# tjsdn3065/Practice_path_planning_for_formula_student_driverless

Hardware: AMD Instinct MI355X
Metric: PGD outer-iters/sec (N=2000 samples, closed, competition_map1, 1024 alpha-seeds/GPU, min-curv) (higher is better)
Workload: dtype f64; 1 GPU; C2: competition_map1 closed, N=2000, B=1024 alpha-seeds per GPU, min-curvature, 14 outer iterations, default cfg::Config; N=2000, batch_per_gpu=1024, global_batch=1024, parallelism=dp1: one GPU, no collective

## Files before the change

### practice_path_planning_for_formula_student_driverless_amd/csrc/rl_optimize_body.inc

```
    constexpr int NW = T / 64;
    constexpr bool WARM = WarmStart<T, MT>::value;
    __shared__ Smem<K, T, WARM> sm;
#ifdef RL_STAMPS
    unsigned long long st_acc[16] = {};
    unsigned long long st_last = __builtin_amdgcn_s_memtime();
#endif

    const int tid = threadIdx.x, lane = tid & 63, wid = tid >> 6;
    const int N = p.N;
    const int base = tid * K;
    const int Ta = (N + K - 1) / K;
    const bool active = tid < Ta;
    const int cnt = RAGGED ? min(K, max(0, N - base)) : (tid < Ta ? K : 0);
    const int cntL = N - (Ta - 1) * K;
    const int wid_u = __builtin_amdgcn_readfirstlane(wid);
    const bool part_wave = RAGGED && (cntL != K) && (((Ta - 1) >> 6) == wid_u);
    const bool tail_wave = wid_u >= ((Ta - 1) >> 6);
    constexpr bool OPEN_FAST = !CLOSED && !RAGGED && K >= 4;
    const bool edge_wave = OPEN_FAST && (wid_u == 0 || wid_u == ((Ta - 1) >> 6));
    const bool fl = tid == 0, ll = tid == Ta - 1;
    const rl_cfg& C = p.cfg[p.ncfg == 1 ? 0 : b];
    const uint64_t seed = p.seeds ? p.seeds[b] : 0ull;

    const double Lb = p.Ls ? p.Ls[RL_BID_] : p.L;
    const double h = uni(Lb / (double)N);
    const double* __restrict__ CEN = p.center + (size_t)RL_BID_ * (size_t)p.center_stride;
    const double invh = uni(1.0 / h), inv2h = uni(1.0 / (2 * h)), invh2 = uni(1.0 / (h * h));
    const double m2invh2 = uni(-2 * invh2);
    const double two_h = uni(2 * h), hh = uni(h * h);
    const double lam = C.lambda_smooth;
    const double lam2 = uni(2.0 * lam);
    const double lam_act = active ? lam : 0.0;
    const bool is_last = tid == Ta - 1;
    const bool wrap_lane = tail_wave && is_last;
    const double step_init = C.step_init, step_min = C.step_min, armijo_c = C.armijo_c;
    const int max_inner = C.max_inner_iters;

    const size_t off = (size_t)b * (size_t)N;
    double* __restrict__ X = p.x + off;
    double* __restrict__ Y = p.y + off;
    double* __restrict__ NX = p.nx + off;
    double* __restrict__ NY = p.ny + off;
    double* __restrict__ ATOT = p.alpha_total + off;
    double* __restrict__ ALAST = p.alpha_last + off;

    double* aF = nullptr;
    double* aL = nullptr;
    double* aW = nullptr;
    if constexpr (NW > 1) {
        aF = &sm.pubF[0][(lane == 0) ? 64 + wid : lane];
        aL = &sm.pubL[0][(lane == 63) ? 64 + wid : lane];
        aW = &sm.pubW[0][(tid == Ta - 1) ? 64 : lane];
    }
    auto xpub = [&](int slot, const double (&a)[K]) RL_AI {
        if constexpr (NW > 1) {
            constexpr int RF = PubTab<NW>::RF;
            const double first = a[0], last = a[K - 1];
            aF[slot * RF] = first;
            aL[slot * RF] = last;
            if (!RAGGED || cntL == K) {
                aW[slot * 65] = last;
            } else if (part_wave) {
                const double lv = pick(a, cntL - 1);
                if (tid == Ta - 1) sm.pubW[slot][64] = lv;
            }
        }
    };
    auto xget = [&](int slot, const double (&a)[K], double& lv, double& rv) RL_AI {
        double el, ef;
        if constexpr (NW == 1) {
            const double lastv = (!RAGGED || cntL == K) ? a[K - 1] : pick(a, cnt - 1);
            el = readlane(lastv, Ta - 1);
            ef = readlane(a[0], 0);
        } else {
            el = (wid > 0) ? sm.pubL[slot][64 + ((wid > 0) ? wid - 1 : 0)] : sm.pubW[slot][64];
            ef = sm.pubF[slot][64 + ((wid + 1 < NW) ? wid + 1 : 0)];
        }
        lv = dpp_from_left_or(a[K - 1], el);
        rv = dpp_from_right_or(a[0], ef);
        if (CLOSED) {
            double e0 = ef;
            if constexpr (NW > 1) e0 = sm.pubF[slot][64];
            rv = wrap_lane ? e0 : rv;
        }
    };
    auto fill_pad = [&](double (&a)[K], double rv) RL_AI {
        if (part_wave && cnt != K && active) {
#pragma unroll
            for (int k = 0; k < K; ++k) a[k] = (k < cnt) ? a[k] : rv;
        }
    };

    constexpr int GHOST_KMAX = 2;
    constexpr bool GHOST = NW > 1 && K <= GHOST_KMAX;
    constexpr bool VSPLIT = MT && K == 1 && NW >= 2 && T <= 512;
    constexpr bool SPEC = GHOST;
    constexpr int KT = K * T;
    __shared__ double gq[GHOST ? 2 * 3 * KT : 1];
    __shared__ double gred[GHOST ? 2 * 2 * NW : 1];
    auto wrapj = [&](int j) RL_AI -> int {
        if (CLOSED) { j %= N; return j < 0 ? j + N : j; }
        return j < 0 ? 0 : (j >= N ? N - 1 : j);
    };
    const int jl2 = wrapj(base - 2), jl1 = wrapj(base - 1), jr1 = wrapj(base + cnt), jr2 = wrapj(base + cnt + 1);
    double cL = 0.0, gL = 0.0, loL = 0.0, hiL = 0.0, tL = 0.0;
    double cR = 0.0, gR = 0.0, loR = 0.0, hiR = 0.0, tR = 0.0;
    int gpar = 0, gpar_last = 0;

    auto loadP = [&](double (&px)[K + 4], double (&py)[K + 4]) RL_AI {
        const int bs = opaque(base);
        if (bs >= 2 && bs + K + 2 <= N) {
            const double* xb = X + (bs - 2);
            const double* yb = Y + (bs - 2);
#pragma unroll
            for (int j = 0; j < K + 4; ++j) { px[j] = xb[j]; py[j] = yb[j]; }
        } else {
#pragma unroll
            for (int j = 0; j < K + 4; ++j) {
                int g = bs - 2 + j;
                if (CLOSED) { g %= N; if (g < 0) g += N; }
                else g = g < 0 ? 0 : (g >= N ? N - 1 : g);
                px[j] = X[g];
                py[j] = Y[g];
            }
        }
    };
    auto own = [&](int k) RL_AI -> int { return min(opaque(base) + k, N - 1); };
    auto deriv = [&](const double (&px)[K + 4], const double (&py)[K + 4], int k, double& xp, double& yp,
                     double& xpp, double& ypp) RL_AI {
        const int i = base + k;
        if (N == 1) { xp = 1; yp = 0; xpp = ypp = 0; return; }
        if (CLOSED) {
            xp = (px[k + 3] - px[k + 1]) / two_h; yp = (py[k + 3] - py[k + 1]) / two_h;
            xpp = (sub2x(px[k + 3], px[k + 2]) + px[k + 1]) / hh; ypp = (sub2x(py[k + 3], py[k + 2]) + py[k + 1]) / hh;
        } else if (i == 0) {
            xp = (px[k + 3] - px[k + 2]) / h; yp = (py[k + 3] - py[k + 2]) / h;
            if (N >= 3) { xpp = (sub2x(px[k + 4], px[k + 3]) + px[k + 2]) / hh; ypp = (sub2x(py[k + 4], py[k + 3]) + py[k + 2]) / hh; }
            else xpp = ypp = 0;
        } else if (i == N - 1) {
            xp = (px[k + 2] - px[k + 1]) / h; yp = (py[k + 2] - py[k + 1]) / h;
            if (N >= 3) { xpp = (sub2x(px[k + 2], px[k + 1]) + px[k]) / hh; ypp = (sub2x(py[k + 2], py[k + 1]) + py[k]) / hh; }
            else xpp = ypp = 0;
        } else {
            xp = (px[k + 3] - px[k + 1]) / two_h; yp = (py[k + 3] - py[k + 1]) / two_h;
            xpp = (sub2x(px[k + 3], px[k + 2]) + px[k + 1]) / hh; ypp = (sub2x(py[k + 3], py[k + 2]) + py[k + 1]) / hh;
        }
    };
    constexpr bool LDSX = !VSPLIT;
    constexpr bool ALLR = K <= 2;
    constexpr bool A12R = ALLR || (!MT && (CLOSED || K < 8)) || (MT && CLOSED && T >= 256);
    constexpr bool N0R = ALLR || (A12R && !MT);
    constexpr bool WR = ALLR;
    constexpr bool ONCHIP = !MT && CLOSED && K == 8 && A12R && N0R && !WR && LDSX && !GHOST && NW > 1;
    auto normals = [&](const double (&xs)[K], const double (&ys)[K]) RL_AI {
        if (!active) return;
        const double2* pxy = &sm.u.coef[0][0][0];
        double2* pn = &sm.u.coef[1][0][0];
        const int bs = opaque(base);
        const int jl = wrapj(bs - 1), jr = wrapj(bs + cnt);
        const double2 pl = pxy[(jl % K) * T + jl / K], pr = pxy[(jr % K) * T + jr / K];
#pragma unroll
        for (int k = 0; k < K; ++k) {
            const int i = bs + k;
            const double xm = (k > 0) ? xs[k > 0 ? k - 1 : 0] : pl.x, ym = (k > 0) ? ys[k > 0 ? k - 1 : 0] : pl.y;
            double xn = pr.x, yn = pr.y;
            if (k + 1 < K && (!RAGGED || k + 1 < cnt)) { xn = xs[k + 1 < K ? k + 1 : k]; yn = ys[k + 1 < K ? k + 1 : k]; }
            double tx, ty;
            if (N == 1) { tx = 1; ty = 0; }
            else if (CLOSED) { tx = (xn - xm) * 0.5; ty = (yn - ym) * 0.5; }
            else if (i == 0) { tx = xn - xs[k]; ty = yn - ys[k]; }
            else if (i == N - 1) { tx = xs[k] - xm; ty = ys[k] - ym; }
            else { tx = (xn - xm) * 0.5; ty = (yn - ym) * 0.5; }
            if (sqrt(tx * tx + ty * ty) < 1e-15) { tx = 1; ty = 0; }
            double vx = -ty, vy = tx;
            double n = sqrt(vx * vx + vy * vy);
            double ox = 0, oy = 0;
            if (!(n < 1e-15)) { ox = vx / n; oy = vy / n; }
            if constexpr (!ONCHIP) {
                if (k < cnt) { NX[i] = ox; NY[i] = oy; }
            }
            pn[k * T + tid] = make_double2(ox, oy);
        }
    };
    auto normals_kappa = [&](double (&kaout)[K]) RL_AI {
        double px[K + 4], py[K + 4];
        loadP(px, py);
        const int bs = opaque(base);
#pragma unroll
        for (int k = 0; k < K; ++k) {
            const int i = bs + k;
            double tx, ty;
            if (N == 1) { tx = 1; ty = 0; }
            else if (CLOSED) { tx = (px[k + 3] - px[k + 1]) * 0.5; ty = (py[k + 3] - py[k + 1]) * 0.5; }
            else if (i == 0) { tx = px[k + 3] - px[k + 2]; ty = py[k + 3] - py[k + 2]; }
            else if (i == N - 1) { tx = px[k + 2] - px[k + 1]; ty = py[k + 2] - py[k + 1]; }
            else { tx = (px[k + 3] - px[k + 1]) * 0.5; ty = (py[k + 3] - py[k + 1]) * 0.5; }
            if (sqrt(tx * tx + ty * ty) < 1e-15) { tx = 1; ty = 0; }
            double vx = -ty, vy = tx;
            double n = sqrt(vx * vx + vy * vy);
            double ox = 0, oy = 0;
            if (!(n < 1e-15)) { ox = vx / n; oy = vy / n; }
            if (active && k < cnt) { NX[i] = ox; NY[i] = oy; }
            double xp, yp, xpp, ypp;
            deriv(px, py, k, xp, yp, xpp, ypp);
            const double kav = (xp * ypp - yp * xpp) / pow15(smax(1e-12, xp * xp + yp * yp));
            kaout[k] = (active && k < cnt) ? kav : 0.0;
        }
    };
    constexpr int CKK = CK < K ? CK : K;
    auto corridor_scan = [&](double guard, bool pre) RL_AI {
        double2* bnd = &sm.u.coef[0][0][0];
        for (int c = (NW == 1) ? 0 : -1;; c = (NW == 1) ? c + 1 : -1) {
            if constexpr (NW > 1) {
                int q = 0;
                if (lane == 0) q = atomicAdd(&sm.ctr, 1);
                c = __builtin_amdgcn_readlane(q, 0);
            }
            if (c * 64 * CKK >= N) break;
            const int i0 = (c * 64 + lane) * CKK;
            double qx[CKK], qy[CKK], ux[CKK], uy[CKK], lc[CKK], hc[CKK];
            bool act[CKK];
#pragma unroll
            for (int k = 0; k < CKK; ++k) {
                const int i = min(i0 + k, N - 1);
                if constexpr (LDSX) {
                    const double2 q = bnd[(i % K) * T + i / K], u = sm.u.coef[1][i % K][i / K];
                    qx[k] = q.x; qy[k] = q.y; ux[k] = u.x; uy[k] = u.y;
                } else {
                    qx[k] = X[i]; qy[k] = Y[i]; ux[k] = NX[i]; uy[k] = NY[i];
                }
                act[k] = i0 + k < N;
            }
            if (pre) {
#pragma unroll
                for (int k = 0; k < CKK; ++k) {
                    const int i = min(i0 + k, N - 1);
                    lc[k] = p.lo0[i];
                    hc[k] = p.hi0[i];
                }
            } else {
#ifdef RL_STAMPS
            RL_STAMP(7);
            corridor_bounds<CKK, false>(p.ring[0], p.ring[1], qx, qy, ux, uy, act, guard,
                                                                      lc, hc, [&](int s) { RL_STAMP(s); });
#else
            corridor_bounds<CKK, false>(p.ring[0], p.ring[1], qx, qy, ux, uy, act, guard,
                                                                      lc, hc);
#endif
            }
#pragma unroll
            for (int k = 0; k < CKK; ++k) {
                const int i = i0 + k;
                if (act[k]) bnd[(i % K) * T + i / K] = make_double2(lc[k], hc[k]);
            }
        }
    };
    auto corridor_collect = [&](double (&lo)[K], double (&hi)[K]) RL_AI {
        const double2* bnd = &sm.u.coef[0][0][0];
        __syncthreads();
#pragma unroll
        for (int k = 0; k < K; ++k) {
            const double2 v = bnd[k * T + tid];
            lo[k] = (k < cnt) ? v.x : 0.0;
            hi[k] = (k < cnt) ? v.y : 0.0;
        }
        if constexpr (GHOST) {
            const double2 vl = bnd[(jl1 % K) * T + jl1 / K], vr = bnd[(jr1 % K) * T + jr1 / K];
            loL = vl.x; hiL = vl.y; loR = vr.x; hiR = vr.y;
        }
        __syncthreads();
    };
    auto corridor = [&](double guard, bool pre, double (&lo)[K], double (&hi)[K]) RL_AI {
        corridor_scan(guard, pre);
        corridor_collect(lo, hi);
    };

    if (tid == 0) {
        VConst vc;
        const double a_total = C.use_total_ge_lat ? smax(C.a_total_max, C.a_lat_max) : C.a_total_max;
        vc.a_total2 = a_total * a_total;
        vc.kFd = 0.5 * C.rho_air * C.Cd * C.A_front_m2;
        vc.Fr = C.mass_kg * 9.81 * C.c_rr;
        vc.mass = C.mass_kg; vc.Pmax = C.P_max_W;
        vc.acc_cap = vs_cap(C.a_long_acc_cap); vc.brk_cap = vs_cap(C.a_long_brake_cap);
        vc.h = h;
        vc.pw_free = power_never_binds(C.P_max_W, C.mass_kg, vc.kFd, vc.Fr, C.v_cap_mps, vc.acc_cap);
        sm.vc = vc;
    }
    if constexpr (WARM) {
#pragma unroll
        for (int j = 0; j < 4; ++j) sm.vg[j][tid] = INFINITY;
    }

    auto same_bits = [](double a, double b) RL_AI -> bool { return __double_as_longlong(a) == __double_as_longlong(b); };
    auto vpass = [&](const double (&ka)[K], double (&v)[K]) RL_AI -> int {
        const VConst vc = vconst_uniform(sm.vc);
#pragma unroll
        for (int k = 0; k < K; ++k) {
            double kk = fabs(ka[k]);
            double v_kappa = sqrt(C.a_lat_max / smax(kk, C.kappa_eps));
            v[k] = (k < cnt) ? smin(C.v_cap_mps, v_kappa) : INFINITY;
        }
        const int iters = C.max_vpass_iters;
        int sweeps = 0;
        const bool has_right = active && (base + cnt < N);
        const bool has_left = active && (base > 0);
        for (int s = 0; s < iters; ++s) {
            ++sweeps;
            double vstart[K];
#pragma unroll
            for (int k = 0; k < K; ++k) vstart[k] = v[k];
            {
                double g = INFINITY;
                if constexpr (WARM) g = sm.vg[s == 0 ? 0 : 1][tid];
                double in_prev = -1.0;
                double out = INFINITY;
                double wave_in = g;
                double pub = -1.0;
                bool first = true;
                for (int ro = 0;; ++ro) {
                    bool conv = false;
                    for (int ir = 0; ir < VpRounds<K, T>::value; ++ir) {
                        double in = dpp_from_left_or(out, wave_in);
                        if (first) in = g;
                        if (!has_left) in = INFINITY;
                        bool ch = false;
                        if (active && in != in_prev) {
                            in_prev = in;
                            double cur = vstart[0];
                            if (has_left) cur = smin(vstart[0], in);
                            bool go = first || !same_bits(cur, v[0]);
                            v[0] = cur;
#pragma unroll
                            for (int k = 0; k + 1 < K; ++k) {
                                if (!__any(go)) break;
                                if (go) {
                                    const double vf = vstep_fwd(vc, v[k], ka[k]);
                                    const double nv = (k + 1 < cnt) ? smin(vstart[k + 1], vf) : INFINITY;
                                    go = first || !same_bits(nv, v[k + 1]);
                                    v[k + 1] = nv;
                                }
                            }
                            if (has_right && go) {
                                const double o = vstep_fwd(vc, v[K - 1], ka[K - 1]);
                                ch = o != out;
                                out = o;
                            }
                        }
                        if (first) { first = false; continue; }
                        if (!__any(ch)) { conv = true; break; }
                    }
                    if constexpr (NW == 1) break;
                    bool pch = false;
                    if (lane == 63 && has_right) {
                        pch = out != pub;
                        pub = out;
                        sm.u.vin[ro & 1][wid] = out;
                    }
                    if (!__syncthreads_or(pch || !conv) && ro > 0) break;
                    if (wid > 0) wave_in = sm.u.vin[ro & 1][wid - 1];
                }
                if constexpr (WARM) {
                    sm.vg[1][tid] = in_prev;
                    if (s == 0) sm.vg[0][tid] = in_prev;
                }
            }
            if (CLOSED) {
                if (active && base + cnt == N) {
                    double vl = (cnt == K) ? v[K - 1] : pick(v, cnt - 1);
                    double kl = (cnt == K) ? ka[K - 1] : pick(ka, cnt - 1);
                    sm.bc[0] = vstep_fwd(vc, vl, kl);
                }
                __syncthreads();
                if (tid == 0) v[0] = smin(v[0], sm.bc[0]);
                __syncthreads();
            }
            {
                double vpre[K];
#pragma unroll
                for (int k = 0; k < K; ++k) vpre[k] = v[k];
                double g = INFINITY;
                if constexpr (WARM) g = sm.vg[s == 0 ? 2 : 3][tid];
                double in_prev = -1.0;
                double out = INFINITY;
                double wave_in = g;
                double pub = -1.0;
                bool first = true;
                for (int ro = 0;; ++ro) {
                    bool conv = false;
                    for (int ir = 0; ir < VpRounds<K, T>::value; ++ir) {
                        double in = dpp_from_right_or(out, wave_in);
                        if (first) in = g;
                        if (!has_right) in = INFINITY;
                        bool ch = false;
                        if (active && in != in_prev) {
                            in_prev = in;
                            const double cur = has_right ? smin(vpre[K - 1], in) : vpre[K - 1];
                            bool go = first || !same_bits(cur, v[K - 1]);
                            v[K - 1] = cur;
#pragma unroll
                            for (int k = K - 2; k >= 0; --k) {
                                if (!__any(go)) break;
                                if (go) {
                                    const double vb = vstep_bwd(vc, v[k + 1], ka[k + 1]);
                                    const double nv = (k < cnt) ? smin(vpre[k], vb) : INFINITY;
                                    go = first || !same_bits(nv, v[k]);
                                    v[k] = nv;
                                }
                            }
                            if (has_left && go) {
                                const double o = vstep_bwd(vc, v[0], ka[0]);
                                ch = o != out;
                                out = o;
                            }
                        }
                        if (first) { first = false; continue; }
                        if (!__any(ch)) { conv = true; break; }
                    }
                    if constexpr (NW == 1) break;
                    bool pch = false;
                    if (lane == 0 && has_left) {
                        pch = out != pub;
                        pub = out;
                        sm.u.vin[ro & 1][wid] = out;
                    }
                    if (!__syncthreads_or(pch || !conv) && ro > 0) break;
                    if (wid + 1 < NW) wave_in = sm.u.vin[ro & 1][wid + 1];
                }
                if constexpr (WARM) {
                    sm.vg[3][tid] = in_prev;
                    if (s == 0) sm.vg[2][tid] = in_prev;
                }
            }
            if (CLOSED) {
                if (tid == 0) sm.bc[1] = vstep_bwd(vc, v[0], ka[0]);
                __syncthreads();
                if (active && base + cnt == N) {
                    if (cnt == K) v[K - 1] = smin(v[K - 1], sm.bc[1]);
                    else put(v, cnt - 1, smin(pick(v, cnt - 1), sm.bc[1]));
                }
                __syncthreads();
            }
            bool any_change = false;
#pragma unroll
            for (int k = 0; k < K; ++k) any_change |= (k < cnt) && (v[k] != vstart[k]);
            if (!__syncthreads_or(any_change)) break;
        }
        return sweeps;
    };

    constexpr int KP = VSPLIT ? T / 64 : 1;
    __shared__ double vsv[VSPLIT ? T : 1];
    double vwg[4] = {INFINITY, INFINITY, INFINITY, INFINITY};
    auto vpass1w = [&]() RL_AI -> int {
        const VConst vc = vconst_uniform(sm.vc);
        const int b0 = lane * KP;
        const int c1 = min(KP, max(0, N - b0));
        double ka1[KP], v[KP];
#pragma unroll
        for (int j = 0; j < KP; ++j) {
            ka1[j] = (j < c1) ? vsv[b0 + j] : 0.0;
            const double kk = fabs(ka1[j]);
            const double v_kappa = sqrt(C.a_lat_max / smax(kk, C.kappa_eps));
            v[j] = (j < c1) ? smin(C.v_cap_mps, v_kappa) : INFINITY;
        }
        const bool act1 = c1 > 0, hasL = act1 && b0 > 0, hasR = act1 && b0 + c1 < N;
        const int lastl = (N - 1) / KP;
        const int iters = C.max_vpass_iters;
        int sweeps = 0;
        for (int s = 0; s < iters; ++s) {
            ++sweeps;
            double vstart[KP];
#pragma unroll
            for (int j = 0; j < KP; ++j) vstart[j] = v[j];
            {
                const double g = vwg[s == 0 ? 0 : 1];
                double in_prev = -1.0, out = INFINITY;
                bool first = true;
                for (;;) {
                    double in = dpp_from_left_or(out, INFINITY);
                    if (first) in = g;
                    if (!hasL) in = INFINITY;
                    bool ch = false;
                    if (act1 && in != in_prev) {
                        in_prev = in;
                        double cur = vstart[0];
                        if (hasL) cur = smin(vstart[0], in);
                        bool go = first || !same_bits(cur, v[0]);
                        v[0] = cur;
#pragma unroll
                        for (int j = 0; j + 1 < KP; ++j) {
                            if (!__any(go)) break;
                            if (go) {
                                const double vf = vstep_fwd(vc, v[j], ka1[j]);
                                const double nv = (j + 1 < c1) ? smin(vstart[j + 1], vf) : INFINITY;
                                go = first || !same_bits(nv, v[j + 1]);
                                v[j + 1] = nv;
                            }
                        }
                        if (hasR && go) {
                            const double o = vstep_fwd(vc, v[KP - 1], ka1[KP - 1]);
                            ch = o != out;
                            out = o;
                        }
                    }
                    if (first) { first = false; continue; }
                    if (!__any(ch)) break;
                }
                vwg[1] = in_prev;
                if (s == 0) vwg[0] = in_prev;
            }
            if (CLOSED) {
                const double f = readlane(vstep_fwd(vc, pick(v, c1 - 1), pick(ka1, c1 - 1)), lastl);
                if (lane == 0) v[0] = smin(v[0], f);
            }
            {
                double vpre[KP];
#pragma unroll
                for (int j = 0; j < KP; ++j) vpre[j] = v[j];
                const double g = vwg[s == 0 ? 2 : 3];
                double in_prev = -1.0, out = INFINITY;
                bool first = true;
                for (;;) {
                    double in = dpp_from_right_or(out, INFINITY);
                    if (first) in = g;
                    if (!hasR) in = INFINITY;
                    bool ch = false;
                    if (act1 && in != in_prev) {
                        in_prev = in;
                        const double cur = hasR ? smin(vpre[KP - 1], in) : vpre[KP - 1];
                        bool go = first || !same_bits(cur, v[KP - 1]);
                        v[KP - 1] = cur;
#pragma unroll
                        for (int j = KP - 2; j >= 0; --j) {
                            if (!__any(go)) break;
                            if (go) {
                                const double vb = vstep_bwd(vc, v[j + 1], ka1[j + 1]);
                                const double nv = (j < c1) ? smin(vpre[j], vb) : INFINITY;
                                go = first || !same_bits(nv, v[j]);
                                v[j] = nv;
                            }
                        }
                        if (hasL && go) {
                            const double o = vstep_bwd(vc, v[0], ka1[0]);
                            ch = o != out;
                            out = o;
                        }
                    }
                    if (first) { first = false; continue; }
                    if (!__any(ch)) break;
                }
                vwg[3] = in_prev;
                if (s == 0) vwg[2] = in_prev;
            }
            if (CLOSED) {
                const double f = readlane(vstep_bwd(vc, v[0], ka1[0]), 0);
                if (lane == lastl) put(v, c1 - 1, smin(pick(v, c1 - 1), f));
            }
            bool any_change = false;
#pragma unroll
            for (int j = 0; j < KP; ++j) any_change |= (j < c1) && (v[j] != vstart[j]);
            if (!__any(any_change)) break;
        }
#pragma unroll
        for (int j = 0; j < KP; ++j)
            if (j < c1) vsv[b0 + j] = v[j];
        return sweeps;
    };

    auto d1_at = [&](int k, double am, double a0, double ap) RL_AI -> double {
        if (CLOSED) return (ap - am) * inv2h;
        const int i = base + k;
        if (N == 1) return 0.0;
        if (i == 0) return (ap - a0) * invh;
        if (i == N - 1) return (a0 - am) * invh;
        return (ap - am) * inv2h;
    };
    auto d2_at = [&](int k, double am, double a0, double ap) RL_AI -> double {
        if (CLOSED) return (sub2x(ap, a0) + am) * invh2;
        const int i = base + k;
        if (N <= 2 || i == 0 || i == N - 1) return 0.0;
        return (sub2x(ap, a0) + am) * invh2;
    };
    auto d1t_at = [&](int k, double vm, double v0, double vp) RL_AI -> double {
        if (CLOSED) return (vm - vp) * inv2h;
        const int j = base + k;
        if (N <= 1) return 0.0;
        double acc = 0.0;
        if (j >= 1) acc += ((j == 1) ? invh : inv2h) * vm;
        if (j == 0) acc += (-invh) * v0;
        else if (j == N - 1) acc += (+invh) * v0;
        if (j <= N - 2) acc += ((j + 1 == N - 1) ? -invh : -inv2h) * vp;
        return acc;
    };

    const double inv2h_x2 = uni(2.0 * inv2h), invh_x2 = uni(2.0 * invh), invh2_x2 = uni(2.0 * invh2),
                 m2invh2_x2 = uni(2.0 * m2invh2);
    auto d1t_x2 = [&](int k, double vm, double v0, double vp) RL_AI -> double {
        if (CLOSED) return (vm - vp) * inv2h_x2;
        const int j = base + k;
        if (N <= 1) return 0.0;
        double acc = 0.0;
        if (j >= 1) acc += ((j == 1) ? invh_x2 : inv2h_x2) * vm;
        if (j == 0) acc += (-invh_x2) * v0;
        else if (j == N - 1) acc += (+invh_x2) * v0;
        if (j <= N - 2) acc += ((j + 1 == N - 1) ? -invh_x2 : -inv2h_x2) * vp;
        return acc;
    };
    auto d2t_x2 = [&](int k, double vm, double v0, double vp) RL_AI -> double {
        if (CLOSED) return (sub2x(vp, v0) + vm) * invh2_x2;
        const int j = base + k;
        if (N <= 2) return 0.0;
        double acc = 0.0;
        if (j - 1 >= 1 && j - 1 <= N - 2) acc += (+invh2_x2) * vm;
        if (j >= 1 && j <= N - 2) acc += m2invh2_x2 * v0;
        if (j + 1 >= 1 && j + 1 <= N - 2) acc += (+invh2_x2) * vp;
        return acc;
    };
    auto grad_at = [&](int k, double q1m, double q10, double q1p, double q2m, double q20, double q2p, double am,
                       double a0, double ap) RL_AI -> double {
        double g1 = d1t_x2(k, q1m, q10, q1p);
        double g2 = d2t_x2(k, q2m, q20, q2p);
        double gsm = d1t_at(k, am, a0, ap);
        return (g1 + g2) + lam2 * gsm;
    };
    auto grad_int = [&](double q1m, double q1p, double q2m, double q20, double q2p, double am, double ap) RL_AI
        -> double {
        const double g1 = (0.0 + inv2h_x2 * q1m) + (-inv2h_x2) * q1p;
        const double g2 = ((0.0 + invh2_x2 * q2m) + m2invh2_x2 * q20) + invh2_x2 * q2p;
        const double gsm = (0.0 + inv2h * am) + (-inv2h) * ap;
        return (g1 + g2) + lam2 * gsm;
    };

    double G2[K];
    double lo[K], hi[K], al[K], gr[K], an[K];
    double q1[K], q2[K], a1v[K];
    double A1r[K], A2r[K], N0r[K], Wr[K];

    auto part_dec = [&](const double (&a)[K], const double (&cur)[K], const double (&g)[K]) RL_AI -> double {
        double pdec = 0.0;
        if (part_wave) {
#pragma unroll
            for (int k = 0; k < K; ++k)
                if (k < cnt) pdec = __builtin_fma(g[k], a[k] - cur[k], pdec);
        } else {
#pragma unroll
            for (int k = 0; k < K; ++k) pdec = __builtin_fma(g[k], a[k] - cur[k], pdec);
        }
        return pdec;
    };
    auto eval_part = [&](double (&a)[K], double lv, double rv) RL_AI -> double {
        fill_pad(a, rv);
        double pJ = 0.0, pJsm = 0.0;
        double jr[K];
#pragma unroll
        for (int k = 0; k < K; ++k) {
            const double2 c01 = A12R ? make_double2(A1r[k], A2r[k]) : sm.u.coef[0][k][tid];
            const double2 c23 = WR ? make_double2(N0r[k], Wr[k])
                                : N0R ? make_double2(N0r[k], sm.u.coef[1][k][tid].y) : sm.u.coef[1][k][tid];
            double am = (k > 0) ? a[k - 1] : lv;
            double ap = (k + 1 < K) ? a[k + 1] : rv;
            double x1, x2;
            if (OPEN_FAST && edge_wave && (k == 0 || k == K - 1)) {
                const bool e = (k == 0) ? fl : ll;
                const double om = (k == 0 && fl) ? a[k] : am;
                const double op = (k == K - 1 && ll) ? a[k] : ap;
                x1 = (op - om) * (e ? invh : inv2h);
                const double x2i = (sub2x(ap, a[k]) + am) * invh2;
                x2 = e ? 0.0 : x2i;
            } else if (OPEN_FAST) {
                x1 = (ap - am) * inv2h;
                x2 = (sub2x(ap, a[k]) + am) * invh2;
            } else {
                x1 = d1_at(k, am, a[k], ap);
                x2 = d2_at(k, am, a[k], ap);
            }
            double r = c23.y * (c23.x + c01.x * x1 + c01.y * x2);
            jr[k] = r;
            double Wz = MT ? (c23.y * G2[k] * r) : (c23.y * r);
            q1[k] = c01.x * Wz;
            q2[k] = c01.y * Wz;
            a1v[k] = x1;
        }
        auto acc = [&](int k) RL_AI {
            pJ = __builtin_fma(MT ? G2[k] * jr[k] : jr[k], jr[k], pJ);
            pJsm = __builtin_fma(a1v[k], a1v[k], pJsm);
        };
        if (part_wave) {
#pragma unroll
            for (int k = 0; k < K; ++k)
                if (k < cnt) acc(k);
        } else {
#pragma unroll
            for (int k = 0; k < K; ++k) acc(k);
        }
        pJ = __builtin_fma(lam_act, pJsm, pJ);
        if constexpr (GHOST) {
            double* const Q = &gq[gpar * 3 * KT];
#pragma unroll
            for (int k = 0; k < K; ++k) { Q[base + k] = q1[k]; Q[KT + base + k] = q2[k]; Q[2 * KT + base + k] = a1v[k]; }
        } else {
            xpub(1, q1);
            xpub(2, q2);
            xpub(3, a1v);
        }
        return pJ;
    };
    auto eval_j = [&](double (&a)[K], const double (&cur)[K], const double (&g)[K], bool trial,
                      double& dec) RL_AI -> double {
        const double pdec = trial ? part_dec(a, cur, g) : 0.0;
        double lv, rv;
        RL_ESTAMP(11);
        if constexpr (GHOST) {
            lv = trial ? tL : cL;
            rv = trial ? tR : cR;
        } else {
            xpub(0, a);
            if constexpr (NW > 1) __syncthreads();
            xget(0, a, lv, rv);
        }
        const double pJ = eval_part(a, lv, rv);
        RL_ESTAMP(12);
        const double z = wave_sum_xy(pJ, pdec, lane & 1);
        RL_ESTAMP(13);
        if constexpr (NW == 1) {
            dec = readlane(z, 1);
            return readlane(z, 0);
        }
        if constexpr (GHOST) {
            double* const R = &gred[gpar * 2 * NW];
            if (lane < 2) R[lane * NW + wid] = z;
            __syncthreads();
            double J = R[0], D = R[NW];
#pragma unroll
            for (int w = 1; w < NW; ++w) { J += R[w]; D += R[NW + w]; }
            dec = D;
            gpar_last = gpar;
            gpar ^= 1;
            RL_ESTAMP(14);
            return J;
        }
        if (lane < 2) sm.red[lane][wid] = z;
        __syncthreads();
        double J = sm.red[0][0], D = sm.red[1][0];
#pragma unroll
        for (int w = 1; w < NW; ++w) { J += sm.red[0][w]; D += sm.red[1][w]; }
        dec = D;
        return J;
    };
    auto eval_grad = [&](double (&g)[K]) RL_AI {
        double l1, r1, l2, r2, l3, r3;
        if constexpr (GHOST) {
            const double* const Q = &gq[gpar_last * 3 * KT];
            l1 = Q[jl1]; r1 = Q[jr1]; l2 = Q[KT + jl1]; r2 = Q[KT + jr1]; l3 = Q[2 * KT + jl1]; r3 = Q[2 * KT + jr1];
            const double q1a = (!RAGGED || cnt == K) ? q1[K - 1] : pick(q1, cnt > 0 ? cnt - 1 : 0);
            const double q2a = (!RAGGED || cnt == K) ? q2[K - 1] : pick(q2, cnt > 0 ? cnt - 1 : 0);
            const double a1a = (!RAGGED || cnt == K) ? a1v[K - 1] : pick(a1v, cnt > 0 ? cnt - 1 : 0);
            gL = grad_at(-1, Q[jl2], l1, q1[0], Q[KT + jl2], l2, q2[0], Q[2 * KT + jl2], l3, a1v[0]);
            gR = grad_at(cnt, q1a, r1, Q[jr2], q2a, r2, Q[KT + jr2], a1a, r3, Q[2 * KT + jr2]);
        } else {
            xget(1, q1, l1, r1);
            xget(2, q2, l2, r2);
            xget(3, a1v, l3, r3);
        }
        fill_pad(q1, r1);
        fill_pad(q2, r2);
        fill_pad(a1v, r3);
#pragma unroll
        for (int k = 0; k < K; ++k) {
            const double q1m = (k > 0) ? q1[k - 1] : l1, q1p = (k + 1 < K) ? q1[k + 1] : r1;
            const double q2m = (k > 0) ? q2[k - 1] : l2, q2p = (k + 1 < K) ? q2[k + 1] : r2;
            const double am = (k > 0) ? a1v[k - 1] : l3, ap = (k + 1 < K) ? a1v[k + 1] : r3;
            if (OPEN_FAST && edge_wave && (k < 2 || k >= K - 2)) {
                const bool e = (k < 2) ? fl : ll;
                double c1A = inv2h_x2, o1A = q1m, c1C = -inv2h_x2, o1C = q1p;
                double o2A = q2m, o2B = q2[k], o2C = q2p;
                double csA = inv2h, osA = am, csC = -inv2h, osC = ap;
                if (k == 0) {
                    c1A = e ? -invh_x2 : c1A; o1A = e ? q1[k] : o1A;
                    o2A = e ? 0.0 : o2A; o2B = e ? 0.0 : o2B;
                    csA = e ? -invh : csA; osA = e ? a1v[k] : osA;
                } else if (k == 1) {
                    c1A = e ? invh_x2 : c1A;
                    o2A = e ? 0.0 : o2A;
                    csA = e ? invh : csA;
                } else if (k == K - 2) {
                    c1C = e ? -invh_x2 : c1C;
                    o2C = e ? 0.0 : o2C;
                    csC = e ? -invh : csC;
                } else {
                    c1C = e ? invh_x2 : c1C; o1C = e ? q1[k] : o1C;
                    o2B = e ? 0.0 : o2B; o2C = e ? 0.0 : o2C;
                    csC = e ? invh : csC; osC = e ? a1v[k] : osC;
                }
                const double g1 = (0.0 + c1A * o1A) + c1C * o1C;
                const double g2 = ((0.0 + invh2_x2 * o2A) + m2invh2_x2 * o2B) + invh2_x2 * o2C;
                const double gsm = (0.0 + csA * osA) + csC * osC;
                g[k] = (g1 + g2) + lam2 * gsm;
            } else if (OPEN_FAST) {
                g[k] = grad_int(q1m, q1p, q2m, q2[k], q2p, am, ap);
            } else {
                g[k] = grad_at(k, q1m, q1[k], q1p, q2m, q2[k], q2p, am, a1v[k], ap);
            }
        }
    };

    const int MO = C.max_outer_iters;
    if (active) {
#pragma unroll
        for (int k = 0; k < K; ++k) {
            if (k < cnt) {
                X[base + k] = CEN[2 * (base + k)];
                Y[base + k] = CEN[2 * (base + k) + 1];
                if (MO == 0) {
                    ATOT[base + k] = 0.0;
                    ALAST[base + k] = 0.0;
                }
            }
        }
    }
#pragma unroll
    for (int k = 0; k < K; ++k) { al[k] = 0.0; gr[k] = 0.0; G2[k] = 0.0; }

    RL_STAMP(0);
    for (int outer = 0;; ++outer) {
#if RL_PRIO
        progress_prio(outer, MO, RL_PRIO);
#endif
        double xs[K], ys[K];
#pragma unroll
        for (int k = 0; k < K; ++k) { xs[k] = 0.0; ys[k] = 0.0; }
        double atot[ONCHIP ? K : 1] = {};
        if (LDSX && outer == 0 && active) {
            const int bu = opaque(base);
#pragma unroll
            for (int k = 0; k < K; ++k)
                if (k < cnt) { xs[k] = CEN[2 * (bu + k)]; ys[k] = CEN[2 * (bu + k) + 1]; }
        }
        if (outer > 0 && active) {
            const int bu = opaque(base);
            const bool last_upd = outer == MO, first_upd = outer == 1;
#pragma unroll
            for (int k = 0; k < K; ++k) {
                if (k < cnt) {
                    const int i = bu + k;
                    if (last_upd) ALAST[i] = al[k];
                    if constexpr (ONCHIP) {
                        const double2 nk = sm.u.coef[0][k][tid];
                        xs[k] = X[i] + nk.x * al[k];
                        ys[k] = Y[i] + nk.y * al[k];
                        X[i] = xs[k];
                        Y[i] = ys[k];
                        double at = 0.0;
                        if (!first_upd) at = sm.u.coef[1][k][tid].x;
                        atot[k] = at + al[k];
                        if (last_upd) ATOT[i] = atot[k];
                    } else {
                        xs[k] = X[i] + NX[i] * al[k];
                        ys[k] = Y[i] + NY[i] * al[k];
                        X[i] = xs[k];
                        Y[i] = ys[k];
                        double at = 0.0;
                        if (!first_upd) at = ATOT[i];
                        ATOT[i] = at + al[k];
                    }
                }
            }
        }
        if (LDSX && outer < MO) {
#pragma unroll
            for (int k = 0; k < K; ++k) sm.u.coef[0][k][tid] = make_double2(xs[k], ys[k]);
        }
#pragma unroll
        for (int k = 0; k < K; ++k) { al[k] = 0.0; gr[k] = 0.0; }
        cL = cR = gL = gR = 0.0;
        __syncthreads();
        RL_STAMP(5);
        auto seed_alpha = [&]() RL_AI {
            if (outer == 0 && seed != 0) {
#pragma unroll
                for (int k = 0; k < K; ++k) {
                    double s0 = seed_value(seed, opaque(base) + k, RL_SEED_SIGMA);
                    al[k] = (k < cnt) ? smin(hi[k], smax(lo[k], s0)) : 0.0;
                }
                if constexpr (GHOST) {
                    cL = smin(hiL, smax(loL, seed_value(seed, jl1, RL_SEED_SIGMA)));
                    cR = smin(hiR, smax(loR, seed_value(seed, jr1, RL_SEED_SIGMA)));
                }
            }
        };
        const double guard = (outer == 0 ? p.veh_width : C.veh_width_m) * 0.5 + C.safety_margin_m;
        const bool pre = outer == 0 && p.lo0 != nullptr;
        double ka[K];
        bool ka_done = false;
        if (outer < MO) {
            if (tid == 0) sm.ctr = 0;
            if constexpr (VSPLIT) {
                normals_kappa(ka);
                vsv[tid] = ka[0];
                ka_done = true;
            } else {
                normals(xs, ys);
            }
            __syncthreads();
            if constexpr (!VSPLIT) {
#if defined(RL_STAMPS) && !defined(RL_STAMPS_EVAL)
                RL_STAMP(11);
#endif
                corridor(guard, pre, lo, hi);
                seed_alpha();
            }
        }
        RL_STAMP(1);
        if ((MT || outer == MO) && !ka_done) {
            double hd[K];
            double px[K + 4], py[K + 4];
            loadP(px, py);
#pragma unroll
            for (int k = 0; k < K; ++k) {
                double xp, yp, xpp, ypp;
                deriv(px, py, k, xp, yp, xpp, ypp);
                double hdv = (outer == MO) ? atan2_noinline(yp, xp) : 0.0;
                double denom = pow15(smax(1e-12, xp * xp + yp * yp));
                double kav = (xp * ypp - yp * xpp) / denom;
                hd[k] = (k < cnt) ? hdv : 0.0;
                ka[k] = (k < cnt) ? kav : 0.0;
                __builtin_amdgcn_sched_barrier(0);
            }
            if (outer == MO && active) {
#pragma unroll
                for (int k = 0; k < K; ++k)
                    if (k < cnt) { p.heading[off + opaque(base) + k] = hd[k]; p.kappa[off + opaque(base) + k] = ka[k]; }
            }
        }
        if (MT) {
            double v[K];
            if constexpr (VSPLIT) {
                if (!ka_done) {
                    vsv[tid] = ka[0];
                    __syncthreads();
                }
                RL_STAMP(2);
                if (wid_u == NW - 1) {
                    const int sw = vpass1w();
                    if (lane == 0 && p.sweeps) p.sweeps[(size_t)b * (MO + 1) + outer] = sw;
#if defined(RL_STAMPS) && !defined(RL_STAMPS_EVAL)
                    RL_STAMP(12);
#endif
                    if (outer < MO) corridor_scan(guard, pre);
                } else if (outer < MO) {
#if defined(RL_STAMPS) && !defined(RL_STAMPS_EVAL)
                    const unsigned long long ts0 = __builtin_amdgcn_s_memtime();
                    corridor_scan(guard, pre);
                    if (wid_u < 3) st_acc[13 + wid_u] += __builtin_amdgcn_s_memtime() - ts0;
#else
                    corridor_scan(guard, pre);
#endif
                }
                if (outer < MO) {
                    corridor_collect(lo, hi);
                    seed_alpha();
                } else {
                    __syncthreads();
                }
#if defined(RL_STAMPS) && !defined(RL_STAMPS_EVAL)
                RL_STAMP(11);
#endif
                v[0] = active ? vsv[tid] : INFINITY;
            } else {
                const int sw = vpass(ka, v);
                if (tid == 0 && p.sweeps) p.sweeps[(size_t)b * (MO + 1) + outer] = sw;
            }
            if (outer == MO) {
                double lv, rv;
                xpub(0, v);
                __syncthreads();
                xget(0, v, lv, rv);
                double lt = 0.0;
                if (active) {
#pragma unroll
                    for (int k = 0; k < K; ++k) {
                        if (k < cnt) {
                            const int i = base + k;
                            double v1;
                            if (i + 1 < N) v1 = (k + 1 < cnt) ? v[(k + 1 < K) ? k + 1 : k] : rv;
                            else v1 = CLOSED ? rv : v[k];
                            double v0 = v[k];
                            p.ax[off + i] = (v1 * v1 - v0 * v0) / two_h;
                            p.v[off + i] = v0;
                            lt += h / smax(1e-6, v[k]);
                        }
                    }
                }
                lt = wave_sum(lt);
                if (lane == 0) sm.red2[1][wid] = lt;
                __syncthreads();
                if (tid == 0 && p.lap) {
                    double tot = sm.red2[1][0];
                    for (int w = 1; w < NW; ++w) tot += sm.red2[1][w];
                    p.lap[b] = tot;
                }
            } else {
                double v_avg = 0.0;
                if (C.time_weight_use_inv_v) {
                    double vs = 0.0;
#pragma unroll
                    for (int k = 0; k < K; ++k) if (k < cnt) vs += v[k];
                    vs = wave_sum(vs);
                    if (lane == 0) sm.red2[0][wid] = vs;
                    __syncthreads();
                    double tot = sm.red2[0][0];
                    for (int w = 1; w < NW; ++w) tot += sm.red2[0][w];
                    v_avg = tot / (double)(N > 1 ? N : 1);
                }
#pragma unroll
                for (int k = 0; k < K; ++k) {
                    double kk = fabs(ka[k]);
                    double vkappa = sqrt(C.a_lat_max / smax(kk, C.kappa_eps));
                    double rr = smin(1.0, v[k] / smax(1e-6, vkappa));
                    double r = rr * rr;
                    r = smin(1.0, smax(0.0, r));
                    double rp;
                    if (C.time_gamma_power == 2.0) rp = r * r;
                    else rp = pow_noinline(r, C.time_gamma_power);
                    double corner_w = 1.0 + C.w_time_gain * rp;
                    double invv_w = 1.0;
                    if (C.time_weight_use_inv_v) {
                        double ratio = v_avg / smax(1e-6, v[k]);
                        invv_w = 1.0 + C.inv_v_gain * (ratio - 1.0);
                        if (invv_w < 1.0) invv_w = 1.0;
                        if (invv_w > 3.0) invv_w = 3.0;
                    }
                    double gamma = corner_w * invv_w;
                    G2[k] = (k < cnt) ? gamma * gamma : 0.0;
                }
                __syncthreads();
            }
        }
        RL_STAMP(2);
        if (outer == MO) break;

        {
            double px[K + 4], py[K + 4];
            loadP(px, py);
#pragma unroll
            for (int k = 0; k < K; ++k) {
                double xp, yp, xpp, ypp;
                deriv(px, py, k, xp, yp, xpp, ypp);
                double nxk, nyk;
                if constexpr (ONCHIP) {
                    const double2 nk = sm.u.coef[1][k][tid];
                    nxk = nk.x; nyk = nk.y;
                    sm.u.coef[0][k][tid] = nk;
                } else {
                    const int i = own(k);
                    nxk = NX[i]; nyk = NY[i];
                }
                double a1 = nxk * ypp - nyk * xpp;
                double a2 = xp * nyk - yp * nxk;
                double n0 = xp * ypp - yp * xpp;
                double denom = pow15(smax(1e-12, xp * xp + yp * yp));
                double w = 1.0 / denom;
                const bool v = k < cnt;
                if (A12R) { A1r[k] = v ? a1 : 0.0; A2r[k] = v ? a2 : 0.0; }
                if (N0R) N0r[k] = v ? n0 : 0.0;
                else sm.u.coef[0][k][tid] = make_double2(v ? a1 : 0.0, v ? a2 : 0.0);
                if (WR) Wr[k] = v ? w : 0.0;
                else if constexpr (ONCHIP) sm.u.coef[1][k][tid] = make_double2(atot[k], v ? w : 0.0);
                else sm.u.coef[1][k][tid] = make_double2(v ? n0 : 0.0, v ? w : 0.0);
            }
        }
        RL_STAMP(3);
        bool zb_lane = false;
#pragma unroll
        for (int k = 0; k < K; ++k)
            zb_lane |= (__double_as_longlong(lo[k]) == (long long)0x8000000000000000ull) ||
                       (hi[k] == 0.0 && k < cnt);
        const bool zb = __builtin_amdgcn_ballot_w64(zb_lane) != 0;
        double step = step_init;
        auto project = [&](const double (&cur)[K], const double (&g)[K], double (&nxt)[K]) RL_AI {
            double ai[K];
#pragma unroll
            for (int k = 0; k < K; ++k) ai[k] = cur[k] - step * g[k];
            if (!zb) {
#pragma unroll
                for (int k = 0; k < K; ++k) nxt[k] = vmin_f64(hi[k], vmax_f64(lo[k], ai[k]));
            } else {
#pragma unroll
                for (int k = 0; k < K; ++k) nxt[k] = smin(hi[k], smax(lo[k], ai[k]));
            }
            if constexpr (GHOST) {
                tL = smin(hiL, smax(loL, cL - step * gL));
                tR = smin(hiR, smax(loR, cR - step * gR));
            }
        };
        double dec;
        double J = eval_j(al, al, gr, false, dec);
        eval_grad(gr);
        int evals = 1, accepts = 0, it = 0;
        double J_prev = J;
        auto inner = [&](const double (&cur)[K], double (&g)[K], double (&nxt)[K]) RL_AI -> int {
            if (it >= max_inner) return 0;
            ++it;
            int bt = 0;
            if constexpr (SPEC) {
                for (;;) {
                    project(cur, g, nxt);
                    double Jn = eval_j(nxt, cur, g, true, dec);
                    ++evals;
                    double gt[K];
                    const double gL0 = gL, gR0 = gR;
                    eval_grad(gt);
#pragma unroll
                    for (int k = 0; k < K; ++k) pin(gt[k]);
                    pin(gL);
                    pin(gR);
                    RL_ESTAMP(15);
                    if (Jn <= J + armijo_c * dec) {
#pragma unroll
                        for (int k = 0; k < K; ++k) g[k] = gt[k];
                        cL = tL; cR = tR;
                        J = Jn;
                        ++accepts;
                        break;
                    }
                    gL = gL0; gR = gR0;
                    step *= 0.5;
                    bt++;
                    if (step < step_min || bt >= 20) return 0;
                }
                if (fabs(J_prev - J) < 1e-10) return 1;
                J_prev = J;
                return 2;
            }
            for (;;) {
                project(cur, g, nxt);
                double Jn = eval_j(nxt, cur, g, true, dec);
                ++evals;
                if (Jn <= J + armijo_c * dec) {
                    eval_grad(g);
                    if constexpr (GHOST) { cL = tL; cR = tR; }
                    J = Jn;
                    ++accepts;
                    break;
                }
                step *= 0.5;
                bt++;
                if (step < step_min || bt >= 20) return 0;
            }
            if (fabs(J_prev - J) < 1e-10) return 1;
            J_prev = J;
            return 2;
        };
        bool in_an = false;
        for (;;) {
            int r = inner(al, gr, an);
            if (r != 2) { in_an = (r == 1); break; }
            r = inner(an, gr, al);
            if (r != 2) { in_an = (r == 0); break; }
        }
        if (in_an) {
#pragma unroll
            for (int k = 0; k < K; ++k) al[k] = an[k];
        }
        if (tid == 0) {
            if (p.evals) p.evals[(size_t)b * MO + outer] = evals;
            if (p.accepts) p.accepts[(size_t)b * MO + outer] = accepts;
        }
        RL_STAMP(4);
    }
    if (p.done) signal_done(p.done, b, p.epoch);
#ifdef RL_STAMPS
    RL_STAMP(6);
    if (tid == 0 && b < 16384) {
        for (int i = 0; i < 16; ++i)
            if (!(VSPLIT && (i == 12 || i == 14 || i == 15))) rl_dbg_stamps[b][i] = st_acc[i];
    }
    if (VSPLIT && lane == 0 && b < 16384) {
        if (wid == NW - 1) rl_dbg_stamps[b][12] = st_acc[12];
        else if (wid == 1 || wid == 2) rl_dbg_stamps[b][13 + wid] = st_acc[13 + wid];
    }
#endif
```

Before: 1.878 million PGD outer-iters/s.

## Keep path coordinates in LDS/registers and recompute normals on the ONCHIP path

```diff
diff --git a/practice_path_planning_for_formula_student_driverless_amd/csrc/rl_optimize_body.inc b/practice_path_planning_for_formula_student_driverless_amd/csrc/rl_optimize_body.inc
--- a/practice_path_planning_for_formula_student_driverless_amd/csrc/rl_optimize_body.inc
+++ b/practice_path_planning_for_formula_student_driverless_amd/csrc/rl_optimize_body.inc
@@ -152,34 +152,59 @@
     constexpr bool N0R = ALLR || (A12R && !MT);
     constexpr bool WR = ALLR;
     constexpr bool ONCHIP = !MT && CLOSED && K == 8 && A12R && N0R && !WR && LDSX && !GHOST && NW > 1;
-    auto normals = [&](const double (&xs)[K], const double (&ys)[K]) RL_AI {
+    constexpr int PA = ONCHIP ? 1 : 0, NA = 1 - PA;
+    auto normal_of = [&](int k, int i, const double (&xs)[K], const double (&ys)[K], const double2 pl, const double2 pr,
+                         double& ox, double& oy) RL_AI {
+        const double xm = (k > 0) ? xs[k > 0 ? k - 1 : 0] : pl.x, ym = (k > 0) ? ys[k > 0 ? k - 1 : 0] : pl.y;
+        double xn = pr.x, yn = pr.y;
+        if (k + 1 < K && (!RAGGED || k + 1 < cnt)) { xn = xs[k + 1 < K ? k + 1 : k]; yn = ys[k + 1 < K ? k + 1 : k]; }
+        double tx, ty;
+        if (N == 1) { tx = 1; ty = 0; }
+        else if (CLOSED) { tx = (xn - xm) * 0.5; ty = (yn - ym) * 0.5; }
+        else if (i == 0) { tx = xn - xs[k]; ty = yn - ys[k]; }
+        else if (i == N - 1) { tx = xs[k] - xm; ty = ys[k] - ym; }
+        else { tx = (xn - xm) * 0.5; ty = (yn - ym) * 0.5; }
+        if (sqrt(tx * tx + ty * ty) < 1e-15) { tx = 1; ty = 0; }
+        double vx = -ty, vy = tx;
+        double n = sqrt(vx * vx + vy * vy);
+        ox = 0; oy = 0;
+        if (!(n < 1e-15)) { ox = vx / n; oy = vy / n; }
+    };
+    auto halo1 = [&](int area, int bs, double2& pl, double2& pr) RL_AI {
+        const double2* pxy = &sm.u.coef[area][0][0];
+        const int jl = wrapj(bs - 1), jr = wrapj(bs + cnt);
+        pl = pxy[(jl % K) * T + jl / K];
+        pr = pxy[(jr % K) * T + jr / K];
+    };
+    auto normals = [&](const double (&xs)[K], const double (&ys)[K], double2& hl, double2& hr) RL_AI {
         if (!active) return;
-        const double2* pxy = &sm.u.coef[0][0][0];
-        double2* pn = &sm.u.coef[1][0][0];
+        const double2* pxy = &sm.u.coef[PA][0][0];
+        double2* pn = &sm.u.coef[NA][0][0];
         const int bs = opaque(base);
         const int jl = wrapj(bs - 1), jr = wrapj(bs + cnt);
         const double2 pl = pxy[(jl % K) * T + jl / K], pr = pxy[(jr % K) * T + jr / K];
+        if constexpr (ONCHIP) { hl = pl; hr = pr; }
 #pragma unroll
         for (int k = 0; k < K; ++k) {
             const int i = bs + k;
-            const double xm = (k > 0) ? xs[k > 0 ? k - 1 : 0] : pl.x, ym = (k > 0) ? ys[k > 0 ? k - 1 : 0] : pl.y;
-            double xn = pr.x, yn = pr.y;
-            if (k + 1 < K && (!RAGGED || k + 1 < cnt)) { xn = xs[k + 1 < K ? k + 1 : k]; yn = ys[k + 1 < K ? k + 1 : k]; }
-            double tx, ty;
-            if (N == 1) { tx = 1; ty = 0; }
-            else if (CLOSED) { tx = (xn - xm) * 0.5; ty = (yn - ym) * 0.5; }
-            else if (i == 0) { tx = xn - xs[k]; ty = yn - ys[k]; }
-            else if (i == N - 1) { tx = xs[k] - xm; ty = ys[k] - ym; }
-            else { tx = (xn - xm) * 0.5; ty = (yn - ym) * 0.5; }
-            if (sqrt(tx * tx + ty * ty) < 1e-15) { tx = 1; ty = 0; }
-            double vx = -ty, vy = tx;
-            double n = sqrt(vx * vx + vy * vy);
-            double ox = 0, oy = 0;
-            if (!(n < 1e-15)) { ox = vx / n; oy = vy / n; }
+            double ox, oy;
+            normal_of(k, i, xs, ys, pl, pr, ox, oy);
             if constexpr (!ONCHIP) {
                 if (k < cnt) { NX[i] = ox; NY[i] = oy; }
             }
             pn[k * T + tid] = make_double2(ox, oy);
+        }
+    };
+    auto regP = [&](const double (&xs)[K], const double (&ys)[K], const double2 pl, const double2 pr, double (&px)[K + 4],
+                    double (&py)[K + 4]) RL_AI {
+        static_assert(!ONCHIP || CLOSED, "deriv's open boundary forms read the halo of 2");
+        px[0] = px[1] = pl.x; py[0] = py[1] = pl.y;
+        px[K + 2] = px[K + 3] = pr.x; py[K + 2] = py[K + 3] = pr.y;
+#pragma unroll
+        for (int k = 0; k < K; ++k) {
+            const bool own_k = !RAGGED || k < cnt;
+            px[k + 2] = own_k ? xs[k] : pr.x;
+            py[k + 2] = own_k ? ys[k] : pr.y;
         }
     };
     auto normals_kappa = [&](double (&kaout)[K]) RL_AI {
@@ -209,7 +234,7 @@
     };
     constexpr int CKK = CK < K ? CK : K;
     auto corridor_scan = [&](double guard, bool pre) RL_AI {
-        double2* bnd = &sm.u.coef[0][0][0];
+        double2* bnd = &sm.u.coef[PA][0][0];
         for (int c = (NW == 1) ? 0 : -1;; c = (NW == 1) ? c + 1 : -1) {
             if constexpr (NW > 1) {
                 int q = 0;
@@ -224,7 +249,7 @@
             for (int k = 0; k < CKK; ++k) {
                 const int i = min(i0 + k, N - 1);
                 if constexpr (LDSX) {
-                    const double2 q = bnd[(i % K) * T + i / K], u = sm.u.coef[1][i % K][i / K];
+                    const double2 q = bnd[(i % K) * T + i / K], u = sm.u.coef[NA][i % K][i / K];
                     qx[k] = q.x; qy[k] = q.y; ux[k] = u.x; uy[k] = u.y;
                 } else {
                     qx[k] = X[i]; qy[k] = Y[i]; ux[k] = NX[i]; uy[k] = NY[i];
@@ -256,7 +281,7 @@
         }
     };
     auto corridor_collect = [&](double (&lo)[K], double (&hi)[K]) RL_AI {
-        const double2* bnd = &sm.u.coef[0][0][0];
+        const double2* bnd = &sm.u.coef[PA][0][0];
         __syncthreads();
 #pragma unroll
         for (int k = 0; k < K; ++k) {
@@ -810,8 +835,10 @@
 #pragma unroll
         for (int k = 0; k < K; ++k) {
             if (k < cnt) {
-                X[base + k] = CEN[2 * (base + k)];
-                Y[base + k] = CEN[2 * (base + k) + 1];
+                if (!ONCHIP || MO == 0) {
+                    X[base + k] = CEN[2 * (base + k)];
+                    Y[base + k] = CEN[2 * (base + k) + 1];
+                }
                 if (MO == 0) {
                     ATOT[base + k] = 0.0;
                     ALAST[base + k] = 0.0;
@@ -831,6 +858,7 @@
 #pragma unroll
         for (int k = 0; k < K; ++k) { xs[k] = 0.0; ys[k] = 0.0; }
         double atot[ONCHIP ? K : 1] = {};
+        double2 hl = make_double2(0.0, 0.0), hr = make_double2(0.0, 0.0);
         if (LDSX && outer == 0 && active) {
             const int bu = opaque(base);
 #pragma unroll
@@ -840,21 +868,30 @@
         if (outer > 0 && active) {
             const int bu = opaque(base);
             const bool last_upd = outer == MO, first_upd = outer == 1;
+            double xo[ONCHIP ? K : 1], yo[ONCHIP ? K : 1];
+            double2 ol = make_double2(0.0, 0.0), orr = make_double2(0.0, 0.0);
+            if constexpr (ONCHIP) {
+#pragma unroll
+                for (int k = 0; k < K; ++k) {
+                    const double2 pk = sm.u.coef[0][k][tid];
+                    xo[k] = pk.x; yo[k] = pk.y;
+                }
+                halo1(0, bu, ol, orr);
+            }
 #pragma unroll
             for (int k = 0; k < K; ++k) {
                 if (k < cnt) {
                     const int i = bu + k;
                     if (last_upd) ALAST[i] = al[k];
                     if constexpr (ONCHIP) {
-                        const double2 nk = sm.u.coef[0][k][tid];
-                        xs[k] = X[i] + nk.x * al[k];
-                        ys[k] = Y[i] + nk.y * al[k];
-                        X[i] = xs[k];
-                        Y[i] = ys[k];
+                        double nxk, nyk;
+                        normal_of(k, i, xo, yo, ol, orr, nxk, nyk);
+                        xs[k] = xo[k] + nxk * al[k];
+                        ys[k] = yo[k] + nyk * al[k];
                         double at = 0.0;
                         if (!first_upd) at = sm.u.coef[1][k][tid].x;
                         atot[k] = at + al[k];
-                        if (last_upd) ATOT[i] = atot[k];
+                        if (last_upd) { X[i] = xs[k]; Y[i] = ys[k]; ATOT[i] = atot[k]; }
                     } else {
                         xs[k] = X[i] + NX[i] * al[k];
                         ys[k] = Y[i] + NY[i] * al[k];
@@ -867,9 +904,9 @@
                 }
             }
         }
-        if (LDSX && outer < MO) {
-#pragma unroll
-            for (int k = 0; k < K; ++k) sm.u.coef[0][k][tid] = make_double2(xs[k], ys[k]);
+        if (LDSX && (ONCHIP || outer < MO)) {
+#pragma unroll
+            for (int k = 0; k < K; ++k) sm.u.coef[PA][k][tid] = make_double2(xs[k], ys[k]);
         }
 #pragma unroll
         for (int k = 0; k < K; ++k) { al[k] = 0.0; gr[k] = 0.0; }
@@ -900,7 +937,7 @@
                 vsv[tid] = ka[0];
                 ka_done = true;
             } else {
-                normals(xs, ys);
+                normals(xs, ys, hl, hr);
             }
             __syncthreads();
             if constexpr (!VSPLIT) {
@@ -915,7 +952,12 @@
         if ((MT || outer == MO) && !ka_done) {
             double hd[K];
             double px[K + 4], py[K + 4];
-            loadP(px, py);
+            if constexpr (ONCHIP) {
+                if (active) halo1(PA, opaque(base), hl, hr);
+                regP(xs, ys, hl, hr, px, py);
+            } else {
+                loadP(px, py);
+            }
 #pragma unroll
             for (int k = 0; k < K; ++k) {
                 double xp, yp, xpp, ypp;
@@ -1042,16 +1084,17 @@
 
         {
             double px[K + 4], py[K + 4];
-            loadP(px, py);
+            if constexpr (ONCHIP) regP(xs, ys, hl, hr, px, py);
+            else loadP(px, py);
 #pragma unroll
             for (int k = 0; k < K; ++k) {
                 double xp, yp, xpp, ypp;
                 deriv(px, py, k, xp, yp, xpp, ypp);
                 double nxk, nyk;
                 if constexpr (ONCHIP) {
-                    const double2 nk = sm.u.coef[1][k][tid];
+                    const double2 nk = sm.u.coef[NA][k][tid];
                     nxk = nk.x; nyk = nk.y;
-                    sm.u.coef[0][k][tid] = nk;
+                    sm.u.coef[0][k][tid] = make_double2(xs[k], ys[k]);
                 } else {
                     const int i = own(k);
                     nxk = NX[i]; nyk = NY[i];
```

Result: no change. 1.895 million PGD outer-iters/s (median of 6 runs) (+0.9%).
